# bdwsq1996/Effi-MVS-plus

Measured on AMD Instinct MI355X. Metric: ref-views/sec (cost-volume hot path: warp + cost volume + 3-D regularisation + cascaded GRU refinement), higher is better.
Workload: dtype f32 (3x3 MFMA convs: products as 3 bf16 partial products hi*hi+hi*lo+lo*hi, f32 accumulate; all else f32); 1 GPU; cfg3: DTU-shaped 1600x1184, N=5 views (S=4 sources), 3-stage cascade ndepths=48,8,8, GRU iters 3,3,3, seeded-random weights, features of the stock FPN resident in HBM; parallelism=single GPU, views_in_flight=3, arithmetic=split

## Files before the change

### effi_mvs_plus_amd/csrc/api.hip

```cpp
#include "common.hpp"
#include <cstdlib>
#include <cstring>
#include <mutex>

extern "C" int effi_version(void) { return 200; }

extern "C" const char* effi_error_string(int code) {
    switch (code) {
        case EFFI_OK: return "ok";
        case EFFI_ERR_BADARG: return "bad argument (null pointer, non-positive size, or inconsistent shapes)";
        case EFFI_ERR_UNSUPPORTED: return "shape / channel count not instantiated in this build";
        case EFFI_ERR_LAUNCH: return "kernel launch failed (hipPeekAtLastError)";
        case EFFI_ERR_WORKSPACE: return "no workspace registered for the current device (effi_set_workspace)";
        default: return "unknown error code";
    }
}

static const void* g_workspace[EFFI_MAX_DEVICES];

extern "C" long effi_workspace_bytes(void) { return 256; }

extern "C" int effi_set_workspace(int device, void* workspace, long bytes) {
    if (device < 0 || device >= EFFI_MAX_DEVICES) return EFFI_ERR_BADARG;
    if (workspace != nullptr && bytes < effi_workspace_bytes()) return EFFI_ERR_BADARG;
    __atomic_store_n(&g_workspace[device], (const void*)workspace, __ATOMIC_RELEASE);
    return EFFI_OK;
}

extern "C" const void* effi_get_workspace(int device) {
    if (device < 0 || device >= EFFI_MAX_DEVICES) return nullptr;
    return __atomic_load_n(&g_workspace[device], __ATOMIC_ACQUIRE);
}

const float* effi_zero_page() {
    int dev = -1;
    if (hipGetDevice(&dev) != hipSuccess) return nullptr;
    return (const float*)effi_get_workspace(dev);
}

namespace {
const char* const kOptName[EFFI_OPT_COUNT] = {"warp_lds_kb", "dyn_form", "dyn_setup_exact", "dyn_xchg", "pixnet_mfma", "force_mr", "mr4_min",
                                              "mr4_nt2_max", "mr2_min", "wide_tiles", "roll_mr", "roll_zt", "roll_rp", "deconv_mr", "sr_waves", "enc_gen_mr3", "c3_lean", "dyn_win"};
long g_opt[EFFI_OPT_COUNT];
std::once_flag g_opt_once;
void load_options() {
    for (int i = 0; i < EFFI_OPT_COUNT; ++i) {
        char env[64] = "EFFI_";
        size_t n = strlen(env);
        for (const char* c = kOptName[i]; *c && n + 1 < sizeof(env); ++c) env[n++] = (*c >= 'a' && *c <= 'z') ? (char)(*c - 32) : *c;
        env[n] = 0;
        const char* v = getenv(env);
        g_opt[i] = (v && *v) ? atol(v) : EFFI_OPT_UNSET;
    }
}
int find_option(const char* name) {
    if (!name) return -1;
    for (int i = 0; i < EFFI_OPT_COUNT; ++i)
        if (strcmp(name, kOptName[i]) == 0) return i;
    return -1;
}
}

long effi_option(int id) {
    std::call_once(g_opt_once, load_options);
    return __atomic_load_n(&g_opt[id], __ATOMIC_RELAXED);
}

extern "C" int effi_set_option(const char* name, long value) {
    const int id = find_option(name);
    if (id < 0) return EFFI_ERR_BADARG;
    std::call_once(g_opt_once, load_options);
    __atomic_store_n(&g_opt[id], value, __ATOMIC_RELAXED);
    return EFFI_OK;
}

extern "C" long effi_get_option(const char* name) {
    const int id = find_option(name);
    return id < 0 ? EFFI_OPT_UNSET : effi_option(id);
}

extern "C" long effi_option_unset(void) { return EFFI_OPT_UNSET; }

namespace {
__global__ __launch_bounds__(256) void lds_poison_kernel(unsigned pattern, unsigned* sink) {
    __shared__ unsigned buf[16 * 1024];
    for (int i = threadIdx.x; i < 16 * 1024; i += 256) buf[i] = pattern;
    __syncthreads();
    if (buf[(threadIdx.x * 61) & 16383] != pattern) sink[0] = 1;
}
}

extern "C" int effi_debug_poison_lds(unsigned pattern, void* sink4, effi_stream_t stream) {
    if (!sink4) return EFFI_ERR_BADARG;
    hipLaunchKernelGGL(lds_poison_kernel, dim3(2048), dim3(256), 0, effi_s(stream), pattern, reinterpret_cast<unsigned*>(sink4));
    EFFI_LAUNCH_CHECK();
// ... 63 lines not shown
```

### effi_mvs_plus_amd/csrc/common.hpp

```cpp
#pragma once
#include <hip/hip_runtime.h>
#include "../../include/effi_mvs_hip.h"

#define EFFI_LAUNCH_CHECK()                                   \
    do {                                                      \
        if (hipPeekAtLastError() != hipSuccess) return EFFI_ERR_LAUNCH; \
    } while (0)

const float* effi_zero_page();

enum EffiOption {
    EFFI_OPT_WARP_LDS_KB,
    EFFI_OPT_DYN_FORM,
    EFFI_OPT_DYN_SETUP_EXACT,
    EFFI_OPT_DYN_XCHG,
    EFFI_OPT_PIXNET_MFMA,
    EFFI_OPT_FORCE_MR,
    EFFI_OPT_MR4_MIN, EFFI_OPT_MR4_NT2_MAX, EFFI_OPT_MR2_MIN,
    EFFI_OPT_WIDE_TILES,
    EFFI_OPT_ROLL_MR, EFFI_OPT_ROLL_ZT, EFFI_OPT_ROLL_RP,
    EFFI_OPT_DECONV_MR,
    EFFI_OPT_SR_WAVES,
    EFFI_OPT_ENC_GEN_MR3,
    EFFI_OPT_C3_LEAN,
    EFFI_OPT_DYN_WIN,
    EFFI_OPT_COUNT
};
constexpr long EFFI_OPT_UNSET = -0x7fffffffL;
long effi_option(int id);

static inline hipStream_t effi_s(effi_stream_t s) {
    (void)hipGetLastError();
    return reinterpret_cast<hipStream_t>(s);
}
static inline int effi_cdiv(long a, long b) { return (int)((a + b - 1) / b); }

struct EffiPtrList {
    const float* p[EFFI_MAX_VIEWS + 1];
    const float* const* tbl;
};
__device__ __forceinline__ const float* effi_resolve_views(const float* ref, const EffiPtrList& l) {
    return l.tbl ? l.tbl[0] : ref;
}
struct EffiOutList {
    float* p[EFFI_MAX_VIEWS + 1];
};

__device__ __forceinline__ float effi_dpp_f(float v, int ctrl_sel) {
    int i = __float_as_int(v);
    int r;
    switch (ctrl_sel) {
        case 0:  r = __builtin_amdgcn_update_dpp(0, i, 0xB1, 0xF, 0xF, true); break;
        case 1:  r = __builtin_amdgcn_update_dpp(0, i, 0x4E, 0xF, 0xF, true); break;
        default: r = __builtin_amdgcn_update_dpp(0, i, 0x141, 0xF, 0xF, true); break;
    }
    return __int_as_float(r);
}

template <int LPP>
__device__ __forceinline__ float effi_group_sum(float v) {
    static_assert(LPP == 1 || LPP == 2 || LPP == 4 || LPP == 8, "lanes per pixel");
    if (LPP >= 2) v += effi_dpp_f(v, 0);
    if (LPP >= 4) v += effi_dpp_f(v, 1);
    if (LPP >= 8) v += effi_dpp_f(v, 2);
    return v;
}
template <int LPP>
__device__ __forceinline__ float effi_group_max(float v) {
    if (LPP >= 2) v = fmaxf(v, effi_dpp_f(v, 0));
    if (LPP >= 4) v = fmaxf(v, effi_dpp_f(v, 1));
    if (LPP >= 8) v = fmaxf(v, effi_dpp_f(v, 2));
    return v;
}

__device__ __forceinline__ int effi_xcd_remap(int bid, int nblocks) {
    const int q = nblocks >> 3, r = nblocks & 7;
    const int xcd = bid & 7, idx = bid >> 3;
    const int base = (xcd < r) ? xcd * (q + 1) : r * (q + 1) + (xcd - r) * q;
// ... 307 lines not shown
```

### effi_mvs_plus_amd/csrc/conv2d_x3.hpp

```cpp
#pragma once
#include "common.hpp"

#ifdef EFFI_BF16_ONLY
#define EFFI_FN(name) name##_bf16
#else
#define EFFI_FN(name) name
#endif

#ifndef EFFI_ABL
#define EFFI_ABL 0
#endif
#ifndef EFFI_PIPE_FRAGS
#define EFFI_PIPE_FRAGS 0
#endif

#ifndef EFFI_EPI_BATCH
#define EFFI_EPI_BATCH 1
#endif
#ifndef EFFI_EPI_EARLY_MAX
#define EFFI_EPI_EARLY_MAX 16
#endif
#ifndef EFFI_B_EARLY
#define EFFI_B_EARLY 0
#endif
// ... 152 lines not shown
        }
#pragma unroll
        for (int r = 0; r < 4; ++r) dst[(long)r * hw] = effi_sigmoid_split(v[r]) * (is_z ? 1.0f : hv[r]);
    } else if (EPI == EFFI_EPI_GRU_Q) {
        if (nvalid <= 0) return;
        if (SR && a.aux_q4) {
            const long oq = ((long)(co0 >> 2) * hw + pix) * 4;
            const f32x4 h4 = *reinterpret_cast<const f32x4*>(a.aux0 + oq), z4 = *reinterpret_cast<const f32x4*>(a.aux1 + oq);
            f32x4 g;
#pragma unroll
            for (int r = 0; r < 4; ++r) g[r] = (1.0f - z4[r]) * h4[r] + z4[r] * effi_tanh_split(v[r]);
            *reinterpret_cast<f32x4*>(a.out0 + oq) = g;
            effi_sr_store4(a.out_sr, a.sr_hp, a.sr_wp, co0, y, x, g);
            return;
        }
        const long o = (long)co0 * hw + pix;
        float hv[4], zv[4];
#pragma unroll
        for (int r = 0; r < 4; ++r) {
            hv[r] = a.aux0[o + (long)r * hw];
            zv[r] = a.aux1[o + (long)r * hw];
        }
        f32x4 g;
#pragma unroll
        for (int r = 0; r < 4; ++r) g[r] = (1.0f - zv[r]) * hv[r] + zv[r] * effi_tanh_split(v[r]);
#pragma unroll
        for (int r = 0; r < 4; ++r) a.out0[o + (long)r * hw] = g[r];
        if (SR) effi_sr_store4(a.out_sr, a.sr_hp, a.sr_wp, co0, y, x, g);
    }
}

typedef __bf16 bf16x8 __attribute__((ext_vector_type(8)));

#define EFFI_EPI_K1 6
#define EFFI_EPI_K1UP 8
#define EFFI_EPI_K1HEAD 7
typedef __bf16 bf16x2 __attribute__((ext_vector_type(2)));
typedef float f32x2 __attribute__((ext_vector_type(2)));

__device__ __forceinline__ void split_octet(const f32x4 (&pa)[8], int px, bf16x8& hi, bf16x8& lo) {
#pragma unroll
    for (int e = 0; e < 8; e += 2) {
        const f32x2 x = {pa[e][px], pa[e + 1][px]};
        const bf16x2 h2 = __builtin_convertvector(x, bf16x2);
        const f32x2 hf = __builtin_convertvector(h2, f32x2);
        const bf16x2 l2 = __builtin_convertvector(x - hf, bf16x2);
        hi[e] = h2[0];
        hi[e + 1] = h2[1];
        lo[e] = l2[0];
        lo[e + 1] = l2[1];
    }
}

template <int NT, int MR, int EPI, bool ZB, bool WIDE, bool SR = false, int NW = 4, bool GEN = false, bool REMAP = true>
__device__ __forceinline__ void conv2d_k3_bf16x3_tile(const Conv2dArgs a, int tiles_x, int ntiles, int bid, int nbid, int bidy,
                                                      const EncGenArgs* gp = nullptr, int gmode = 0) {
    constexpr int NTHR = NW * 64;
    static_assert(!GEN || SR, "generated inputs use the split-resident LDS image");
    static_assert(NW == 4 || (SR && NW == 8), "eight waves: split-resident kernels only");
    constexpr int TR = WIDE ? NW : NW * MR, TW = WIDE ? 16 * MR : 16;
    constexpr int AR = TR + 2, AW = SR ? TW + 2 : TW + 8, AQ = AW / 4, XOFF = SR ? 0 : 3, XLEFT = 4, CCH = 16, NKS = 5;
    constexpr int MROW = WIDE ? 0 : AW * 8, MCOL = WIDE ? 16 * 8 : 0;
    constexpr int APIX = AR * AW, NITEMS = (APIX / 4) * 2;
    constexpr int APIXP = SR ? ((APIX + 15) & ~15) : APIX;
    constexpr int NPART = kHiOnly ? 1 : 2;
    constexpr int NUA = SR ? (NPART * 2 * APIXP + NTHR - 1) / NTHR : 1;
    constexpr int NBF = NKS * NT * 2 * 64;
    constexpr int NB4 = (NBF + NTHR - 1) / NTHR;
    static_assert(SR || NITEMS <= 256, "one staging item per thread");
    static_assert(!(SR && ZB), "split-resident maps are 2-D");
    static_assert(EPI != EFFI_EPI_HEAD && EPI != EFFI_EPI_ADD_UP2, "epilogue not instantiated for the split-precision kernel");
    static_assert((EPI != EFFI_EPI_K1 && EPI != EFFI_EPI_K1UP && EPI != EFFI_EPI_K1HEAD) || !ZB, "the fused 1x1 epilogue is 2-D only");
    constexpr bool kHead = EPI == EFFI_EPI_K1HEAD;
    static_assert(!kHead || (SR && !WIDE && !GEN), "the one-launch depth head reads split-resident maps on 16-column tiles");
    __shared__ __attribute__((aligned(16))) unsigned short lds_ah[SR ? NUA * NTHR * 8 : APIX * CCH];
    __shared__ __attribute__((aligned(16))) unsigned short lds_al[SR ? 8 : APIX * CCH];
    __shared__ __attribute__((aligned(16))) unsigned short lds_b[NB4 * NTHR * 8];
    const unsigned short* const lds_al_rd = SR ? lds_ah + 2 * APIXP * 8 : lds_al;
    constexpr int IW7 = (AW + 7 + 1) & ~1, IH7 = AR + 7;
    __shared__ float lds_inv[GEN ? IH7 * IW7 : 1];

    const int tid = threadIdx.x, lane = tid & 63, wv = tid >> 6;
    const int li = lane & 15, lk = lane >> 4;
    const int h = a.h, w = a.w;
    const long hw = (long)h * w;
    const int tile = REMAP ? effi_xcd_remap(bid, nbid) : bid;
    if (tile >= ntiles) return;
    const int ty_ = tile / tiles_x;
    const int x0 = kHead ? (tile - ty_ * tiles_x) * (TW - 2) - 1 : (tile - ty_ * tiles_x) * TW, y0 = kHead ? ty_ * (TR - 2) - 1 : ty_ * TR;
    const int zpl = ZB ? bidy : 0;

    const bool stager = tid < NITEMS;
    const int pq = stager ? tid % (APIX / 4) : 0, soct = stager ? tid / (APIX / 4) : 0;
    const int srow = pq / AQ, sqx = pq - srow * AQ;
    const int sgy = y0 - 1 + srow, sgx = x0 - XLEFT + 4 * sqx;
    const bool s_in = stager & (sgy >= 0) & (sgy < h) & (sgx >= 0) & (sgx < w);
    const int s_off = sgy * w + sgx;
    const int s_lds = (soct * APIX + srow * AW + 4 * sqx) * 8;
    const int s_nv = w - sgx;
    const bool s_part = s_nv < 4;

    f32x4 pa[SR ? NUA : 8];
    const int cin_eff = ZB ? 3 * a.cin : a.cin;
    const int nchunks = (cin_eff + CCH - 1) / CCH;
    const unsigned short* wbf = reinterpret_cast<const unsigned short*>(a.wpack);
    int goff[NUA];
    if (SR && !GEN) {
#pragma unroll
        for (int j = 0; j < NUA; ++j) {
            const int u = tid + j * NTHR;
// ... 111 lines not shown
                    if (!kHiOnly) *reinterpret_cast<effi_bf16x8_t*>(&lds_ah[((1 * 2 + oct) * APIXP + p) * 8]) = lo;
                }
            }
        }
        if (GEN && gmode != 0) {
            const EncGenArgs& g = *gp;
            const int hd = g.hd;
            effi_bf16x8_t wh[2], wl[2];
#pragma unroll
            for (int s_ = 0; s_ < 2; ++s_) {
                const int ky = 4 * s_ + lk;
                float wv8[8];
#pragma unroll
                for (int kx = 0; kx < 8; ++kx) wv8[kx] = (ky < 7 && kx < 7) ? g.w_d1[(ky * 7 + kx) * hd + CCH * ch + li] : 0.0f;
                effi_split8(wv8, wh[s_], wl[s_]);
            }
            float b4[4];
#pragma unroll
            for (int r = 0; r < 4; ++r) b4[r] = g.b_d1[CCH * ch + 4 * lk + r];
            constexpr int NSEG = (APIX + 15) / 16;
            for (int seg = wv; seg < NSEG; seg += NW) {
                const int pr = seg * 16 + li, p = min(pr, APIX - 1);
                const int row = p / AW, col = p - row * AW;
                const int gy = y0 - 1 + row, gx = x0 - 1 + col;
                const bool inside = (gy >= 0) & (gy < h) & (gx >= 0) & (gx < w);
                f32x4 acc = {0.0f, 0.0f, 0.0f, 0.0f};
#pragma unroll
                for (int s_ = 0; s_ < 2; ++s_) {
                    const float* rowp = lds_inv + (row + 4 * s_ + lk) * IW7 + col;
                    float x8[8];
#pragma unroll
                    for (int i = 0; i < 8; ++i) x8[i] = rowp[i];
                    effi_bf16x8_t ah, al;
                    effi_split8(x8, ah, al);
                    acc = __builtin_amdgcn_mfma_f32_16x16x32_bf16(wh[s_], ah, acc, 0, 0, 0);
                    acc = __builtin_amdgcn_mfma_f32_16x16x32_bf16(wl[s_], ah, acc, 0, 0, 0);
                    acc = __builtin_amdgcn_mfma_f32_16x16x32_bf16(wh[s_], al, acc, 0, 0, 0);
                }
                f32x4 v;
#pragma unroll
                for (int r = 0; r < 4; ++r) v[r] = inside ? fmaxf(acc[r] + b4[r], 0.0f) : 0.0f;
                const bf16x4 h4 = __builtin_convertvector(v, bf16x4);
                const bf16x4 l4 = __builtin_convertvector(v - __builtin_convertvector(h4, f32x4), bf16x4);
                if (pr < APIX) {
                    const int e = ((lk >> 1) * APIXP + p) * 8 + (lk & 1) * 4;
                    *reinterpret_cast<bf16x4*>(&lds_ah[e]) = h4;
                    if (!kHiOnly) *reinterpret_cast<bf16x4*>(&lds_ah[2 * APIXP * 8 + e]) = l4;
                }
            }
        }
    };

    f32x4 tb[NB4];
    auto fetch_b = [&](int ch) {
#pragma unroll
        for (int j = 0; j < NB4; ++j) {
            const int u = min(tid + j * NTHR, NBF - 1);
            tb[j] = *reinterpret_cast<const f32x4*>(wbf + ((long)ch * NBF + u) * 8);
        }
    };
    constexpr bool kBEarly = SR && !GEN && EFFI_B_EARLY;
    auto stash = [&](int ch) {
        if (!kBEarly || ch == 0) fetch_b(ch);
        if constexpr (GEN) {
            generate(ch);
        } else if constexpr (SR) {
#pragma unroll
            for (int j = 0; j < NUA; ++j) *reinterpret_cast<f32x4*>(&lds_ah[(tid + j * NTHR) * 8]) = pa[j];
        } else if (stager) {
#pragma unroll
            for (int px = 0; px < 4; ++px) {
                bf16x8 hi, lo;
                split_octet(pa, px, hi, lo);
                *reinterpret_cast<bf16x8*>(&lds_ah[s_lds + px * 8]) = hi;
                if (!kHiOnly) *reinterpret_cast<bf16x8*>(&lds_al[s_lds + px * 8]) = lo;
            }
        }
#pragma unroll
        for (int j = 0; j < NB4; ++j) *reinterpret_cast<f32x4*>(&lds_b[(tid + j * NTHR) * 8]) = tb[j];
    };

    int koff[NKS];
#pragma unroll
    for (int s_ = 0; s_ < NKS; ++s_) {
        const int item = 4 * s_ + lk;
        const int tap = min(item >> 1, 8), oct = item & 1;
        koff[s_] = (((WIDE ? wv : wv * MR) + tap / 3) * AW + li + XOFF + tap % 3 + oct * APIXP) * 8;
    }

    f32x4 acc[MR][NT];
#pragma unroll
    for (int m = 0; m < MR; ++m)
#pragma unroll
        for (int n = 0; n < NT; ++n) acc[m][n] = f32x4{0.0f, 0.0f, 0.0f, 0.0f};

    constexpr bool kBatchT = SR && EFFI_EPI_BATCH != 0 && !(EFFI_ABL & 24) &&
                             (EPI == EFFI_EPI_PLAIN || EPI == EFFI_EPI_GRU_ZR || EPI == EFFI_EPI_GRU_Q);
    constexpr int NZ = (EPI == EFFI_EPI_GRU_ZR) ? NT / 2 : 0;
    constexpr int NH = !kBatchT ? 0 : (EPI == EFFI_EPI_GRU_ZR ? NT - NZ : (EPI == EFFI_EPI_GRU_Q ? NT : 0));
    constexpr int NZQ = (kBatchT && EPI == EFFI_EPI_GRU_Q) ? NT : 0;
    constexpr bool kStateEarly = MR * (NH + NZQ) * 4 <= EFFI_EPI_EARLY_MAX;
    const bool ebatch = kBatchT && (EPI == EFFI_EPI_PLAIN || a.aux_q4);
    f32x4 eb[kBatchT ? NT : 1], eh[MR][NH > 0 ? NH : 1], ez[MR][NZQ > 0 ? NZQ : 1];
    unsigned eqb[MR];
    bool einside[MR];
    auto epi_issue_bias = [&]() {
        if (!ebatch) return;
#pragma unroll
        for (int n = 0; n < NT; ++n) eb[n] = *reinterpret_cast<const f32x4*>(a.bias + n * 16 + 4 * lk);
#pragma unroll
        for (int m = 0; m < MR; ++m) {
            const int x = x0 + li + (WIDE ? 16 * m : 0), y = y0 + (WIDE ? wv : wv * MR + m);
            einside[m] = (y < h) & (x < w);
            eqb[m] = ((unsigned)lk * (unsigned)hw + (einside[m] ? (unsigned)(y * w + x) : 0u)) * 4u;
        }
    };
    auto epi_issue_state = [&]() {
        if (!ebatch) return;
#pragma unroll
        for (int m = 0; m < MR; ++m) {
#pragma unroll
            for (int j = 0; j < NH; ++j) eh[m][j] = *reinterpret_cast<const f32x4*>(a.aux0 + (size_t)(eqb[m] + (unsigned)j * 16u * (unsigned)hw));
#pragma unroll
            for (int j = 0; j < NZQ; ++j) ez[m][j] = *reinterpret_cast<const f32x4*>(a.aux1 + (size_t)(eqb[m] + (unsigned)j * 16u * (unsigned)hw));
        }
    };

    constexpr bool kK1 = (EPI == EFFI_EPI_K1 || EPI == EFFI_EPI_K1UP || kHead) && !(EFFI_ABL & 24) && EFFI_EPI_BATCH != 0;
    f32x4 kb[kK1 ? NT : 1], kex[kK1 ? MR : 1];
    if constexpr (kK1) {
#pragma unroll
        for (int n = 0; n < NT; ++n) kb[n] = *reinterpret_cast<const f32x4*>(a.bias + n * 16 + 4 * lk);
#pragma unroll
        for (int m = 0; m < MR; ++m) kex[m] = f32x4{0.0f, 0.0f, 0.0f, 0.0f};
        if (EPI == EFFI_EPI_K1 && a.hd > 0) {
#pragma unroll
            for (int m = 0; m < MR; ++m) {
                const int x = x0 + li + (WIDE ? 16 * m : 0), y = y0 + (WIDE ? wv : wv * MR + m);
                const unsigned pix = ((y < h) & (x < w)) ? (unsigned)(y * w + x) : 0u;
#pragma unroll
                for (int r = 0; r < 4; ++r) {
                    const int c = 4 * lk + r;
                    const float t_ = a.aux0[(size_t)((unsigned)min(c, a.hd - 1) * (unsigned)hw + pix)];
                    kex[m][r] = (c < a.hd) ? t_ : 0.0f;
                }
            }
        }
    }

    constexpr bool kBiasQ = !kBatchT && !kK1 && !(EFFI_ABL & 24) && EFFI_EPI_BATCH != 0;
    f32x4 gb[kBiasQ ? NT : 1];
    if constexpr (kBiasQ) {
#pragma unroll
        for (int n = 0; n < NT; ++n) gb[n] = *reinterpret_cast<const f32x4*>(a.bias + n * 16 + 4 * lk);
    }

    prefetch(0);
    epi_issue_bias();
    if (kStateEarly) epi_issue_state();
    stash(0);
    __syncthreads();
    for (int ch = 0; ch < nchunks; ++ch) {
        if (ch + 1 < nchunks) {
            prefetch(ch + 1);
            if (kBEarly) fetch_b(ch + 1);
        }
        constexpr int PIPE = SR ? EFFI_PIPE_FRAGS : 0;
        constexpr int MF = (PIPE == 2) ? (MR + 1) / 2 : MR, MB = MR - MF;
        bf16x8 ahf[PIPE ? 2 : 1][MF], alf[PIPE ? 2 : 1][MF], ahk[MB > 0 ? MB : 1], alk[MB > 0 ? MB : 1], bhb[NT], blb[NT];
        auto load_front = [&](int s_, int buf) {
#pragma unroll
            for (int m = 0; m < MF; ++m) {
                ahf[buf][m] = *reinterpret_cast<const bf16x8*>(&lds_ah[koff[s_] + m * (MROW + MCOL)]);
                if (!kHiOnly) alf[buf][m] = *reinterpret_cast<const bf16x8*>(&lds_al_rd[koff[s_] + m * (MROW + MCOL)]);
            }
        };
        auto load_back = [&](int s_) {
// ... 242 lines not shown
        for (int t = 0; t < nt2; ++t) {
            bf16x4 wh[NT + 1], wl[NT + 1];
#pragma unroll
            for (int n = 0; n <= NT; ++n) {
                const long f = ((long)(t * (NT + 1) + n) * 2) * 64 + lane;
                wh[n] = *reinterpret_cast<const bf16x4*>(w2 + f * 4);
                wl[n] = *reinterpret_cast<const bf16x4*>(w2 + (f + 64) * 4);
            }
            const int co = t * 16 + 4 * lk;
            float b2[4];
#pragma unroll
            for (int r = 0; r < 4; ++r) b2[r] = a.disp_range[co + r];
#pragma unroll
            for (int m = 0; m < MR; ++m) {
                f32x4 o = {0.0f, 0.0f, 0.0f, 0.0f};
#pragma unroll
                for (int n = 0; n <= NT; ++n) {
                    o = __builtin_amdgcn_mfma_f32_16x16x16bf16_1k(wh[n], xh[m][n], o, 0, 0, 0);
                    if (!kHiOnly) {
                        o = __builtin_amdgcn_mfma_f32_16x16x16bf16_1k(wl[n], xh[m][n], o, 0, 0, 0);
                        o = __builtin_amdgcn_mfma_f32_16x16x16bf16_1k(wh[n], xl[m][n], o, 0, 0, 0);
                    }
                }
                if (inside[m]) {
                    f32x4 vo;
#pragma unroll
                    for (int r = 0; r < 4; ++r) {
                        float v = o[r] + b2[r];
                        if (a.act == EFFI_ACT_RELU) v = fmaxf(v, 0.0f);
                        vo[r] = v;
                    }
                    if (SR && a.out_sr) {
                        effi_sr_store4(a.out_sr, a.sr_hp, a.sr_wp, co, y0 + (WIDE ? wv : wv * MR + m), x0 + li + (WIDE ? 16 * m : 0), vo);
                    } else {
#pragma unroll
                        for (int r = 0; r < 4; ++r)
                            if (co + r < a.n_range) a.out0[(long)(co + r) * hw + pixm[m]] = vo[r];
                    }
                }
            }
        }
        return;
    }
    if constexpr (kBatchT) if (ebatch) {
        if (!kStateEarly) epi_issue_state();
        const unsigned plane = (unsigned)a.sr_hp * (unsigned)a.sr_wp;
#pragma unroll
        for (int m = 0; m < MR; ++m) {
            if (!einside[m]) continue;
            const int x = x0 + li + (WIDE ? 16 * m : 0), y = y0 + (WIDE ? wv : wv * MR + m);
            const unsigned ub = (unsigned)lk * plane + (unsigned)(y + 1) * (unsigned)a.sr_wp + (unsigned)(x + 1);
#pragma unroll
            for (int n = 0; n < NT; ++n) {
                f32x4 v;
#pragma unroll
                for (int r = 0; r < 4; ++r) v[r] = acc[m][n][r] + eb[n][r];
                if constexpr (EPI == EFFI_EPI_PLAIN) {
                    if (a.act == EFFI_ACT_RELU) {
#pragma unroll
                        for (int r = 0; r < 4; ++r) v[r] = fmaxf(v[r], 0.0f);
                    } else if (a.act != EFFI_ACT_NONE) {
#pragma unroll
                        for (int r = 0; r < 4; ++r) v[r] = apply_act(v[r], a.act);
                    }
                    effi_sr_store4_at(a.out_sr, ub + (unsigned)(4 * n) * plane, lk & 1, v);
                    if (a.out0) {
                        float* dst = a.out0 + (long)(n * 16 + 4 * lk) * a.ostride + (long)y * w + x;
#pragma unroll
                        for (int r = 0; r < 4; ++r) dst[(long)r * a.ostride] = v[r];
                    }
                } else if constexpr (EPI == EFFI_EPI_GRU_ZR) {
                    f32x4 g;
                    if (n < NZ) {
#pragma unroll
                        for (int r = 0; r < 4; ++r) g[r] = effi_sigmoid_split(v[r]) * 1.0f;
                        *reinterpret_cast<f32x4*>(a.out0 + (size_t)(eqb[m] + (unsigned)n * 16u * (unsigned)hw)) = g;
                    } else {
#pragma unroll
                        for (int r = 0; r < 4; ++r) g[r] = effi_sigmoid_split(v[r]) * eh[m][n >= NZ ? n - NZ : 0][r];
                        effi_sr_store4_at(a.out_sr, ub + (unsigned)(4 * (n - NZ)) * plane, lk & 1, g);
                    }
                } else {
                    f32x4 g;
#pragma unroll
                    for (int r = 0; r < 4; ++r) g[r] = (1.0f - ez[m][n][r]) * eh[m][n][r] + ez[m][n][r] * effi_tanh_split(v[r]);
                    *reinterpret_cast<f32x4*>(a.out0 + (size_t)(eqb[m] + (unsigned)n * 16u * (unsigned)hw)) = g;
                    effi_sr_store4_at(a.out_sr, ub + (unsigned)(4 * n) * plane, lk & 1, g);
                }
            }
        }
        return;
    }
#pragma unroll
    for (int m = 0; m < MR; ++m) {
        const int x = x0 + li + (WIDE ? 16 * m : 0);
        const int y = y0 + (WIDE ? wv : wv * MR + m);
        if (y >= h || x >= w) continue;
        const long pix = (long)y * w + x;
#pragma unroll
        for (int n = 0; n < NT; ++n)
            conv_epilogue_store_t<((EPI == EFFI_EPI_K1 || EPI == EFFI_EPI_K1UP || EPI == EFFI_EPI_K1HEAD) ? EFFI_EPI_PLAIN : EPI), SR>(a, acc[m][n], n * 16 + 4 * lk, pix, hw, zpl, y, x,
                                                                                                          kBiasQ ? &gb[n] : nullptr);
    }
}

template <int NT, int MR, int EPI, bool ZB = false, bool WIDE = false, bool SR = false, int NW = 4>
__global__ __launch_bounds__(NW * 64) void conv2d_k3_bf16x3_kernel(const Conv2dArgs a, int tiles_x, int ntiles) {
#ifdef EFFI_STAGGER
    if (SR && gridDim.x > 512) {
        const int slot = (blockIdx.x >> 8) % 3;
        for (int i = 0; i < slot * EFFI_STAGGER; ++i) __builtin_amdgcn_s_sleep(127);
    }
#endif
    conv2d_k3_bf16x3_tile<NT, MR, EPI, ZB, WIDE, SR, NW>(a, tiles_x, ntiles, blockIdx.x, gridDim.x, blockIdx.y);
}

template <int NT, int MR, bool WIDE, bool SR = false, int NW = 4>
__global__ __launch_bounds__(NW * 64) void conv2d_k3_bf16x3_pair_kernel(const Conv2dArgs a0, const Conv2dArgs a1, int tiles_x, int ntiles) {
    if (blockIdx.y == 0) conv2d_k3_bf16x3_tile<NT, MR, EFFI_EPI_PLAIN, false, WIDE, SR, NW>(a0, tiles_x, ntiles, blockIdx.x, gridDim.x, 0);
    else conv2d_k3_bf16x3_tile<NT, MR, EFFI_EPI_PLAIN, false, WIDE, SR, NW>(a1, tiles_x, ntiles, blockIdx.x, gridDim.x, 0);
}

template <int NT, int MR, int EPI, bool WIDE>
__global__ __launch_bounds__(256) void conv2d_k3_bf16x3_batch_kernel(const Conv2dArgs a, const ConvBatch b, int tiles_x, int ntiles) {
    const int t = effi_xcd_remap(blockIdx.y * gridDim.x + blockIdx.x, gridDim.x * gridDim.y);
    const int img = t / ntiles;
    conv2d_k3_bf16x3_tile<NT, MR, EPI, false, WIDE, false, 4, false, false>(conv_batch_image(a, b, img), tiles_x, ntiles, t - img * ntiles,
                                                                           ntiles, 0);
}

template <int NT, int MR, bool WIDE>
__global__ __launch_bounds__(256) void conv2d_k3_bf16x3_encgen_pair_kernel(const Conv2dArgs a0, const Conv2dArgs a1, const EncGenArgs g,
                                                                           int tiles_x, int ntiles) {
    conv2d_k3_bf16x3_tile<NT, MR, EFFI_EPI_PLAIN, false, WIDE, true, 4, true>(blockIdx.y == 0 ? a0 : a1, tiles_x, ntiles, blockIdx.x, gridDim.x, 0, &g,
                                                                             (int)blockIdx.y);
}

static long effi_opt_or(int id, long dflt) {
    const long v = effi_option(id);
    return v == EFFI_OPT_UNSET ? dflt : v;
}
static long effi_mr4_min() { return effi_opt_or(EFFI_OPT_MR4_MIN, 400); }
static long effi_mr4_nt2_max() { return effi_opt_or(EFFI_OPT_MR4_NT2_MAX, 1024); }
static long effi_mr2_min() { return effi_opt_or(EFFI_OPT_MR2_MIN, 400); }
template <int NT, int EPI, bool ZB = false, bool SR = false>
static int launch_bf16x3(const Conv2dArgs& a, hipStream_t st) {
    const long cols = effi_cdiv(a.w, 16);
    const long planes = ZB ? a.zcount : 1;
    const long t4 = cols * effi_cdiv(a.h, 16) * planes, t2 = cols * effi_cdiv(a.h, 8) * planes;
    int mr;
    if (t4 >= effi_mr4_min() && !(NT == 2 && t4 >= effi_mr4_nt2_max())) mr = 4;
    else if (t2 >= effi_mr2_min()) mr = 2;
    else mr = 1;
    const long force = effi_opt_or(EFFI_OPT_FORCE_MR, 0);
    if (force) mr = (int)force;
    const long wide_env = effi_opt_or(EFFI_OPT_WIDE_TILES, -1);
    const bool wide = wide_env >= 0 ? wide_env != 0 : (mr == 4 && a.w >= 512 && !ZB);
    if (wide) {
        const int tiles_x = effi_cdiv(a.w, 16 * mr), ntiles = tiles_x * effi_cdiv(a.h, 4);
        const dim3 grid(ntiles, (unsigned)planes);
        if (mr == 4) hipLaunchKernelGGL((conv2d_k3_bf16x3_kernel<NT, 4, EPI, ZB, true, SR>), grid, dim3(256), 0, st, a, tiles_x, ntiles);
        else if (mr == 2) hipLaunchKernelGGL((conv2d_k3_bf16x3_kernel<NT, 2, EPI, ZB, true, SR>), grid, dim3(256), 0, st, a, tiles_x, ntiles);
        else hipLaunchKernelGGL((conv2d_k3_bf16x3_kernel<NT, 1, EPI, ZB, true, SR>), grid, dim3(256), 0, st, a, tiles_x, ntiles);
        return hipPeekAtLastError() == hipSuccess ? EFFI_OK : EFFI_ERR_LAUNCH;
    }
    if constexpr (SR) {
        const long srw = effi_option(EFFI_OPT_SR_WAVES);
        if ((srw == 8 && mr <= 2) || (srw == EFFI_OPT_UNSET && mr == 1 && NT >= 6)) {
            const int tiles_x = (int)cols, ntiles = tiles_x * effi_cdiv(a.h, 8 * mr);
            const dim3 grid(ntiles, 1);
            if (mr == 2) hipLaunchKernelGGL((conv2d_k3_bf16x3_kernel<NT, 2, EPI, false, false, true, 8>), grid, dim3(512), 0, st, a, tiles_x, ntiles);
            else hipLaunchKernelGGL((conv2d_k3_bf16x3_kernel<NT, 1, EPI, false, false, true, 8>), grid, dim3(512), 0, st, a, tiles_x, ntiles);
            return hipPeekAtLastError() == hipSuccess ? EFFI_OK : EFFI_ERR_LAUNCH;
        }
    }
    const int tiles_x = (int)cols, ntiles = tiles_x * effi_cdiv(a.h, 4 * mr);
    const dim3 grid(ntiles, (unsigned)planes);
    if (mr == 4) hipLaunchKernelGGL((conv2d_k3_bf16x3_kernel<NT, 4, EPI, ZB, false, SR>), grid, dim3(256), 0, st, a, tiles_x, ntiles);
    else if (mr == 2) hipLaunchKernelGGL((conv2d_k3_bf16x3_kernel<NT, 2, EPI, ZB, false, SR>), grid, dim3(256), 0, st, a, tiles_x, ntiles);
    else hipLaunchKernelGGL((conv2d_k3_bf16x3_kernel<NT, 1, EPI, ZB, false, SR>), grid, dim3(256), 0, st, a, tiles_x, ntiles);
    return hipPeekAtLastError() == hipSuccess ? EFFI_OK : EFFI_ERR_LAUNCH;
}

template <int NT, int EPI>
static int launch_bf16x3_batch(const Conv2dArgs& a, const ConvBatch& b, hipStream_t st) {
    const long cols = effi_cdiv(a.w, 16);
    const long t4 = cols * effi_cdiv(a.h, 16) * b.n_img, t2 = cols * effi_cdiv(a.h, 8) * b.n_img;
    int mr;
    if (t4 >= effi_mr4_min() && !(NT == 2 && t4 >= effi_mr4_nt2_max())) mr = 4;
    else if (t2 >= effi_mr2_min()) mr = 2;
    else mr = 1;
    const long force = effi_opt_or(EFFI_OPT_FORCE_MR, 0);
    if (force) mr = (int)force;
    if (mr != 1 && mr != 2 && mr != 4) return EFFI_ERR_BADARG;
    const long wide_env = effi_opt_or(EFFI_OPT_WIDE_TILES, -1);
    const bool wide = wide_env >= 0 ? wide_env != 0 : (mr == 4 && a.w >= 512);
    const int tiles_x = wide ? effi_cdiv(a.w, 16 * mr) : (int)cols, ntiles = tiles_x * effi_cdiv(a.h, wide ? 4 : 4 * mr);
    const dim3 grid(ntiles, (unsigned)b.n_img);
    if (wide) {
        if (mr == 4) hipLaunchKernelGGL((conv2d_k3_bf16x3_batch_kernel<NT, 4, EPI, true>), grid, dim3(256), 0, st, a, b, tiles_x, ntiles);
        else if (mr == 2) hipLaunchKernelGGL((conv2d_k3_bf16x3_batch_kernel<NT, 2, EPI, true>), grid, dim3(256), 0, st, a, b, tiles_x, ntiles);
        else hipLaunchKernelGGL((conv2d_k3_bf16x3_batch_kernel<NT, 1, EPI, true>), grid, dim3(256), 0, st, a, b, tiles_x, ntiles);
    } else {
        if (mr == 4) hipLaunchKernelGGL((conv2d_k3_bf16x3_batch_kernel<NT, 4, EPI, false>), grid, dim3(256), 0, st, a, b, tiles_x, ntiles);
        else if (mr == 2) hipLaunchKernelGGL((conv2d_k3_bf16x3_batch_kernel<NT, 2, EPI, false>), grid, dim3(256), 0, st, a, b, tiles_x, ntiles);
        else hipLaunchKernelGGL((conv2d_k3_bf16x3_batch_kernel<NT, 1, EPI, false>), grid, dim3(256), 0, st, a, b, tiles_x, ntiles);
    }
    return hipPeekAtLastError() == hipSuccess ? EFFI_OK : EFFI_ERR_LAUNCH;
}

template <int NT, int MR>
__global__ __launch_bounds__(256) void conv3d_k3_bf16x3_zb_batch_kernel(const Conv2dArgs a, const ConvBatch b, int tiles_x, int ntiles) {
    conv2d_k3_bf16x3_tile<NT, MR, EFFI_EPI_PLAIN, true, false, false, 4>(conv_batch_image(a, b, blockIdx.z), tiles_x, ntiles, blockIdx.x,
                                                                         gridDim.x, blockIdx.y);
}
template <int NT>
static int launch_bf16x3_zb_batch(const Conv2dArgs& a, const ConvBatch& b, hipStream_t st) {
    const long cols = effi_cdiv(a.w, 16), planes = (long)a.zcount * b.n_img;
    const long t4 = cols * effi_cdiv(a.h, 16) * planes, t2 = cols * effi_cdiv(a.h, 8) * planes;
    int mr;
// ... 104 lines not shown
```

### effi_mvs_plus_amd/ops.py

```python
from __future__ import annotations

import ctypes as C
import functools
import os
import threading

import weakref

import torch

from . import _lib
from ._lib import EffiLibraryError, check

ACT_NONE, ACT_RELU, ACT_SIGMOID, ACT_TANH = 0, 1, 2, 3
EPI_PLAIN, EPI_GRU_ZR, EPI_GRU_Q, EPI_HEAD, EPI_ADD_UP2, EPI_NHWC = 0, 1, 2, 3, 4, 5
EPI_ADD_SHUF2, EPI_NHWC_ADD_SHUF2 = 9, 10
MAX_VIEWS = 12


class KernelProfile:

    def __init__(self, keys=None):
        self.keys = None if keys is None else set(keys)
        self.records = []
# ... 6 lines not shown
                out[key] = out.get(key, 0.0) + acc
                acc = 0.0
            else:
                acc += e0.elapsed_time(e1)
        return out

    def summary(self):
        torch.cuda.synchronize()
        out = {}
        for key, work, e0, e1 in self.records:
            if e0 is None:
                continue
            d = out.setdefault(key, {"launches": 0, "ms": 0.0, "flops": 0.0, "bytes": 0.0})
            d["launches"] += 1
            d["ms"] += e0.elapsed_time(e1)
            d["flops"] += work.get("flops", 0.0)
            d["bytes"] += work.get("bytes", 0.0)
        return out


_PROF = None

PRECISIONS = ("split", "fp32", "bf16")
_PRECISION = os.environ.get("EFFI_MVS_PRECISION", "split")
if _PRECISION not in PRECISIONS:
    raise ValueError(f"EFFI_MVS_PRECISION must be one of {PRECISIONS}, got {_PRECISION!r}")


def set_precision(mode):
    global _PRECISION
    if mode not in PRECISIONS:
        raise ValueError(f"precision must be one of {PRECISIONS}, got {mode!r}")
    _PRECISION = mode


def get_precision():
    return _PRECISION


def uses_split():
    return _PRECISION in ("split", "bf16")


def _x3(name):
    return getattr(_lib.lib(), name + "_bf16" if _PRECISION == "bf16" else name)


_PY_OPTION_DEFAULTS = {"warp_x3": 0, "state_q4": 1, "c1k7_mfma": 1, "k5s2_split": 1, "roll": 1, "conv3d_unaligned_split": 1, "conv3d_s2_split": 1, "fpn_conv0_fused": 1,
                       "fpn_split_head": 1, "csp_pair": 1, "head_taps": 1, "enc_tail": 0, "enc_gen": 1, "reduce_chunk": 2048, "gru_fused": 0, "csp_gen": 0,
                       "head_fused": 1, "head_fused_tile": 0, "clear_fused": 1, "setup_fused": 1, "conf_fused": 1,
                       "fpn_batch": 1}
_PY_OPTS = {k: int(os.environ.get("EFFI_" + k.upper(), v)) for k, v in _PY_OPTION_DEFAULTS.items()}
LIB_OPTIONS = ("warp_lds_kb", "dyn_form", "dyn_setup_exact", "dyn_xchg", "pixnet_mfma", "force_mr", "mr4_min", "mr4_nt2_max", "mr2_min",
               "wide_tiles", "roll_mr", "roll_zt", "roll_rp", "deconv_mr", "sr_waves", "enc_gen_mr3", "c3_lean", "dyn_win")


def option(name):
    return _PY_OPTS[name]


def get_option(name):
    if name in _PY_OPTS:
        return _PY_OPTS[name]
    if name not in LIB_OPTIONS:
        raise KeyError(name)
    L = _lib.lib()
    v = L.effi_get_option(name.encode())
    return None if v == L.effi_option_unset() else int(v)


def set_option(name, value):
    before = get_option(name)
    if name in _PY_OPTS:
        _PY_OPTS[name] = _PY_OPTION_DEFAULTS[name] if value is None else int(value)
    else:
        L = _lib.lib()
        check(L.effi_set_option(name.encode(), L.effi_option_unset() if value is None else int(value)), "effi_set_option")
    return before


class options:

    def __init__(self, **kw):
        self.kw, self.before = kw, {}

    def __enter__(self):
        for k, v in self.kw.items():
            self.before[k] = set_option(k, v)
        return self

    def __exit__(self, *exc):
        for k, v in self.before.items():
            set_option(k, v)
        return False


def set_profile(p):
    global _PROF
    _PROF = p


def get_profile():
    return _PROF


def _call(key, work, fn, *args):
    p = _PROF
# ... 2026 lines not shown
```

Before: 633.6 views/s.

## Split output-channel tiles across blocks for small split-resident GRU convs

After: 636.9 views/s (median of 6 runs). Within noise of the previous version (+0.5%).

```diff
diff --git a/effi_mvs_plus_amd/csrc/api.hip b/effi_mvs_plus_amd/csrc/api.hip
--- a/effi_mvs_plus_amd/csrc/api.hip
+++ b/effi_mvs_plus_amd/csrc/api.hip
@@ -40,7 +40,7 @@
 
 namespace {
 const char* const kOptName[EFFI_OPT_COUNT] = {"warp_lds_kb", "dyn_form", "dyn_setup_exact", "dyn_xchg", "pixnet_mfma", "force_mr", "mr4_min",
-                                              "mr4_nt2_max", "mr2_min", "wide_tiles", "roll_mr", "roll_zt", "roll_rp", "deconv_mr", "sr_waves", "enc_gen_mr3", "c3_lean", "dyn_win"};
+                                              "mr4_nt2_max", "mr2_min", "wide_tiles", "roll_mr", "roll_zt", "roll_rp", "deconv_mr", "sr_waves", "enc_gen_mr3", "c3_lean", "dyn_win", "sr_nsplit"};
 long g_opt[EFFI_OPT_COUNT];
 std::once_flag g_opt_once;
 void load_options() {
diff --git a/effi_mvs_plus_amd/csrc/common.hpp b/effi_mvs_plus_amd/csrc/common.hpp
--- a/effi_mvs_plus_amd/csrc/common.hpp
+++ b/effi_mvs_plus_amd/csrc/common.hpp
@@ -24,6 +24,7 @@
     EFFI_OPT_ENC_GEN_MR3,
     EFFI_OPT_C3_LEAN,
     EFFI_OPT_DYN_WIN,
+    EFFI_OPT_SR_NSPLIT,
     EFFI_OPT_COUNT
 };
 constexpr long EFFI_OPT_UNSET = -0x7fffffffL;
diff --git a/effi_mvs_plus_amd/csrc/conv2d_x3.hpp b/effi_mvs_plus_amd/csrc/conv2d_x3.hpp
--- a/effi_mvs_plus_amd/csrc/conv2d_x3.hpp
+++ b/effi_mvs_plus_amd/csrc/conv2d_x3.hpp
@@ -228,10 +228,14 @@
     }
 }
 
-template <int NT, int MR, int EPI, bool ZB, bool WIDE, bool SR = false, int NW = 4, bool GEN = false, bool REMAP = true>
+template <int NT, int MR, int EPI, bool ZB, bool WIDE, bool SR = false, int NW = 4, bool GEN = false, bool REMAP = true, int NTG = NT>
 __device__ __forceinline__ void conv2d_k3_bf16x3_tile(const Conv2dArgs a, int tiles_x, int ntiles, int bid, int nbid, int bidy,
-                                                      const EncGenArgs* gp = nullptr, int gmode = 0) {
+                                                      const EncGenArgs* gp = nullptr, int gmode = 0, int n0 = 0) {
     constexpr int NTHR = NW * 64;
+    constexpr bool kSplit = NTG != NT;
+    static_assert(!kSplit || (SR && !GEN && !ZB && !WIDE && NTG % NT == 0 &&
+                              (EPI == EFFI_EPI_PLAIN || EPI == EFFI_EPI_GRU_ZR || EPI == EFFI_EPI_GRU_Q)),
+                  "N-split: split-resident plain / GRU epilogues on 16-column tiles");
     static_assert(!GEN || SR, "generated inputs use the split-resident LDS image");
     static_assert(NW == 4 || (SR && NW == 8), "eight waves: split-resident kernels only");
     constexpr int TR = WIDE ? NW : NW * MR, TW = WIDE ? 16 * MR : 16;
@@ -449,11 +453,24 @@
     };
 
     f32x4 tb[NB4];
-    auto fetch_b = [&](int ch) {
+    int boff[kSplit ? NB4 : 1];
+    if constexpr (kSplit) {
 #pragma unroll
         for (int j = 0; j < NB4; ++j) {
             const int u = min(tid + j * NTHR, NBF - 1);
-            tb[j] = *reinterpret_cast<const f32x4*>(wbf + ((long)ch * NBF + u) * 8);
+            const int sn = u >> 7, ks = sn / NT;
+            boff[j] = ((ks * NTG + n0 + (sn - ks * NT)) << 7) + (u & 127);
+        }
+    }
+    auto fetch_b = [&](int ch) {
+#pragma unroll
+        for (int j = 0; j < NB4; ++j) {
+            if constexpr (kSplit) {
+                tb[j] = *reinterpret_cast<const f32x4*>(wbf + ((long)ch * (NKS * NTG * 2 * 64) + boff[j]) * 8);
+            } else {
+                const int u = min(tid + j * NTHR, NBF - 1);
+                tb[j] = *reinterpret_cast<const f32x4*>(wbf + ((long)ch * NBF + u) * 8);
+            }
         }
     };
     constexpr bool kBEarly = SR && !GEN && EFFI_B_EARLY;
@@ -493,8 +510,8 @@
 
     constexpr bool kBatchT = SR && EFFI_EPI_BATCH != 0 && !(EFFI_ABL & 24) &&
                              (EPI == EFFI_EPI_PLAIN || EPI == EFFI_EPI_GRU_ZR || EPI == EFFI_EPI_GRU_Q);
-    constexpr int NZ = (EPI == EFFI_EPI_GRU_ZR) ? NT / 2 : 0;
-    constexpr int NH = !kBatchT ? 0 : (EPI == EFFI_EPI_GRU_ZR ? NT - NZ : (EPI == EFFI_EPI_GRU_Q ? NT : 0));
+    constexpr int NZ = (EPI == EFFI_EPI_GRU_ZR) ? NTG / 2 : 0;
+    constexpr int NH = !kBatchT ? 0 : (EPI == EFFI_EPI_GRU_ZR ? (kSplit ? NT : NT - NZ) : (EPI == EFFI_EPI_GRU_Q ? NT : 0));
     constexpr int NZQ = (kBatchT && EPI == EFFI_EPI_GRU_Q) ? NT : 0;
     constexpr bool kStateEarly = MR * (NH + NZQ) * 4 <= EFFI_EPI_EARLY_MAX;
     const bool ebatch = kBatchT && (EPI == EFFI_EPI_PLAIN || a.aux_q4);
@@ -504,7 +521,7 @@
     auto epi_issue_bias = [&]() {
         if (!ebatch) return;
 #pragma unroll
-        for (int n = 0; n < NT; ++n) eb[n] = *reinterpret_cast<const f32x4*>(a.bias + n * 16 + 4 * lk);
+        for (int n = 0; n < NT; ++n) eb[n] = *reinterpret_cast<const f32x4*>(a.bias + (n0 + n) * 16 + 4 * lk);
 #pragma unroll
         for (int m = 0; m < MR; ++m) {
             const int x = x0 + li + (WIDE ? 16 * m : 0), y = y0 + (WIDE ? wv : wv * MR + m);
@@ -517,9 +534,17 @@
 #pragma unroll
         for (int m = 0; m < MR; ++m) {
 #pragma unroll
-            for (int j = 0; j < NH; ++j) eh[m][j] = *reinterpret_cast<const f32x4*>(a.aux0 + (size_t)(eqb[m] + (unsigned)j * 16u * (unsigned)hw));
-#pragma unroll
-            for (int j = 0; j < NZQ; ++j) ez[m][j] = *reinterpret_cast<const f32x4*>(a.aux1 + (size_t)(eqb[m] + (unsigned)j * 16u * (unsigned)hw));
+            for (int j = 0; j < NH; ++j) {
+                if constexpr (kSplit && EPI == EFFI_EPI_GRU_ZR) {
+                    const int t = n0 + j - NZ;
+                    eh[m][j] = f32x4{0.0f, 0.0f, 0.0f, 0.0f};
+                    if (t >= 0) eh[m][j] = *reinterpret_cast<const f32x4*>(a.aux0 + (size_t)(eqb[m] + (unsigned)t * 16u * (unsigned)hw));
+                } else {
+                    eh[m][j] = *reinterpret_cast<const f32x4*>(a.aux0 + (size_t)(eqb[m] + (unsigned)(n0 + j) * 16u * (unsigned)hw));
+                }
+            }
+#pragma unroll
+            for (int j = 0; j < NZQ; ++j) ez[m][j] = *reinterpret_cast<const f32x4*>(a.aux1 + (size_t)(eqb[m] + (unsigned)(n0 + j) * 16u * (unsigned)hw));
         }
     };
 
@@ -868,6 +893,7 @@
             const unsigned ub = (unsigned)lk * plane + (unsigned)(y + 1) * (unsigned)a.sr_wp + (unsigned)(x + 1);
 #pragma unroll
             for (int n = 0; n < NT; ++n) {
+                const int gn = kSplit ? n0 + n : n;
                 f32x4 v;
 #pragma unroll
                 for (int r = 0; r < 4; ++r) v[r] = acc[m][n][r] + eb[n][r];
@@ -879,29 +905,29 @@
 #pragma unroll
                         for (int r = 0; r < 4; ++r) v[r] = apply_act(v[r], a.act);
                     }
-                    effi_sr_store4_at(a.out_sr, ub + (unsigned)(4 * n) * plane, lk & 1, v);
+                    effi_sr_store4_at(a.out_sr, ub + (unsigned)(4 * gn) * plane, lk & 1, v);
                     if (a.out0) {
-                        float* dst = a.out0 + (long)(n * 16 + 4 * lk) * a.ostride + (long)y * w + x;
+                        float* dst = a.out0 + (long)(gn * 16 + 4 * lk) * a.ostride + (long)y * w + x;
 #pragma unroll
                         for (int r = 0; r < 4; ++r) dst[(long)r * a.ostride] = v[r];
                     }
                 } else if constexpr (EPI == EFFI_EPI_GRU_ZR) {
                     f32x4 g;
-                    if (n < NZ) {
+                    if (gn < NZ) {
 #pragma unroll
                         for (int r = 0; r < 4; ++r) g[r] = effi_sigmoid_split(v[r]) * 1.0f;
-                        *reinterpret_cast<f32x4*>(a.out0 + (size_t)(eqb[m] + (unsigned)n * 16u * (unsigned)hw)) = g;
+                        *reinterpret_cast<f32x4*>(a.out0 + (size_t)(eqb[m] + (unsigned)gn * 16u * (unsigned)hw)) = g;
                     } else {
 #pragma unroll
-                        for (int r = 0; r < 4; ++r) g[r] = effi_sigmoid_split(v[r]) * eh[m][n >= NZ ? n - NZ : 0][r];
-                        effi_sr_store4_at(a.out_sr, ub + (unsigned)(4 * (n - NZ)) * plane, lk & 1, g);
+                        for (int r = 0; r < 4; ++r) g[r] = effi_sigmoid_split(v[r]) * eh[m][kSplit ? n : (n >= NZ ? n - NZ : 0)][r];
+                        effi_sr_store4_at(a.out_sr, ub + (unsigned)(4 * (gn - NZ)) * plane, lk & 1, g);
                     }
                 } else {
                     f32x4 g;
 #pragma unroll
                     for (int r = 0; r < 4; ++r) g[r] = (1.0f - ez[m][n][r]) * eh[m][n][r] + ez[m][n][r] * effi_tanh_split(v[r]);
-                    *reinterpret_cast<f32x4*>(a.out0 + (size_t)(eqb[m] + (unsigned)n * 16u * (unsigned)hw)) = g;
-                    effi_sr_store4_at(a.out_sr, ub + (unsigned)(4 * n) * plane, lk & 1, g);
+                    *reinterpret_cast<f32x4*>(a.out0 + (size_t)(eqb[m] + (unsigned)gn * 16u * (unsigned)hw)) = g;
+                    effi_sr_store4_at(a.out_sr, ub + (unsigned)(4 * gn) * plane, lk & 1, g);
                 }
             }
         }
@@ -915,7 +941,7 @@
         const long pix = (long)y * w + x;
 #pragma unroll
         for (int n = 0; n < NT; ++n)
-            conv_epilogue_store_t<((EPI == EFFI_EPI_K1 || EPI == EFFI_EPI_K1UP || EPI == EFFI_EPI_K1HEAD) ? EFFI_EPI_PLAIN : EPI), SR>(a, acc[m][n], n * 16 + 4 * lk, pix, hw, zpl, y, x,
+            conv_epilogue_store_t<((EPI == EFFI_EPI_K1 || EPI == EFFI_EPI_K1UP || EPI == EFFI_EPI_K1HEAD) ? EFFI_EPI_PLAIN : EPI), SR>(a, acc[m][n], (n0 + n) * 16 + 4 * lk, pix, hw, zpl, y, x,
                                                                                                           kBiasQ ? &gb[n] : nullptr);
     }
 }
@@ -931,6 +957,15 @@
     conv2d_k3_bf16x3_tile<NT, MR, EPI, ZB, WIDE, SR, NW>(a, tiles_x, ntiles, blockIdx.x, gridDim.x, blockIdx.y);
 }
 
+template <int NT, int NTL, int MR, int EPI, int NW>
+__global__ __launch_bounds__(NW * 64) void conv2d_k3_bf16x3_nsplit_kernel(const Conv2dArgs a, int tiles_x, int ntiles) {
+    constexpr int NS = NT / NTL;
+    const int t = effi_xcd_remap(blockIdx.x, gridDim.x);
+    const int tile = t / NS;
+    conv2d_k3_bf16x3_tile<NTL, MR, EPI, false, false, true, NW, false, false, NT>(a, tiles_x, ntiles, tile, ntiles, 0, nullptr, 0,
+                                                                                 (t - tile * NS) * NTL);
+}
+
 template <int NT, int MR, bool WIDE, bool SR = false, int NW = 4>
 __global__ __launch_bounds__(NW * 64) void conv2d_k3_bf16x3_pair_kernel(const Conv2dArgs a0, const Conv2dArgs a1, int tiles_x, int ntiles) {
     if (blockIdx.y == 0) conv2d_k3_bf16x3_tile<NT, MR, EFFI_EPI_PLAIN, false, WIDE, SR, NW>(a0, tiles_x, ntiles, blockIdx.x, gridDim.x, 0);
@@ -959,6 +994,26 @@
 static long effi_mr4_min() { return effi_opt_or(EFFI_OPT_MR4_MIN, 400); }
 static long effi_mr4_nt2_max() { return effi_opt_or(EFFI_OPT_MR4_NT2_MAX, 1024); }
 static long effi_mr2_min() { return effi_opt_or(EFFI_OPT_MR2_MIN, 400); }
+template <int NT, int NTL, int EPI>
+static int launch_bf16x3_nsplit(const Conv2dArgs& a, int mr, int nw, hipStream_t st) {
+    const int tiles_x = effi_cdiv(a.w, 16), ntiles = tiles_x * effi_cdiv(a.h, nw * mr);
+    const dim3 grid((unsigned)ntiles * (NT / NTL), 1);
+    if (nw == 8 && mr == 1) hipLaunchKernelGGL((conv2d_k3_bf16x3_nsplit_kernel<NT, NTL, 1, EPI, 8>), grid, dim3(512), 0, st, a, tiles_x, ntiles);
+    else if (nw == 8 && mr == 2) hipLaunchKernelGGL((conv2d_k3_bf16x3_nsplit_kernel<NT, NTL, 2, EPI, 8>), grid, dim3(512), 0, st, a, tiles_x, ntiles);
+    else if (nw == 4 && mr == 1) hipLaunchKernelGGL((conv2d_k3_bf16x3_nsplit_kernel<NT, NTL, 1, EPI, 4>), grid, dim3(256), 0, st, a, tiles_x, ntiles);
+    else if (nw == 4 && mr == 2) hipLaunchKernelGGL((conv2d_k3_bf16x3_nsplit_kernel<NT, NTL, 2, EPI, 4>), grid, dim3(256), 0, st, a, tiles_x, ntiles);
+    else if (nw == 4 && mr == 4) hipLaunchKernelGGL((conv2d_k3_bf16x3_nsplit_kernel<NT, NTL, 4, EPI, 4>), grid, dim3(256), 0, st, a, tiles_x, ntiles);
+    else return EFFI_ERR_BADARG;
+    return hipPeekAtLastError() == hipSuccess ? EFFI_OK : EFFI_ERR_LAUNCH;
+}
+template <int NT, int EPI>
+static int dispatch_bf16x3_nsplit(const Conv2dArgs& a, int ns, int mr, int nw, hipStream_t st) {
+    if constexpr (NT % 2 == 0) if (ns == 2) return launch_bf16x3_nsplit<NT, NT / 2, EPI>(a, mr, nw, st);
+    if constexpr (NT % 3 == 0) if (ns == 3) return launch_bf16x3_nsplit<NT, NT / 3, EPI>(a, mr, nw, st);
+    if constexpr (NT == 4 || NT == 6) if (ns == NT) return launch_bf16x3_nsplit<NT, 1, EPI>(a, mr, nw, st);
+    return EFFI_ERR_BADARG;
+}
+
 template <int NT, int EPI, bool ZB = false, bool SR = false>
 static int launch_bf16x3(const Conv2dArgs& a, hipStream_t st) {
     const long cols = effi_cdiv(a.w, 16);
@@ -982,6 +1037,20 @@
     }
     if constexpr (SR) {
         const long srw = effi_option(EFFI_OPT_SR_WAVES);
+        if constexpr ((EPI == EFFI_EPI_PLAIN && NT == 3) || (EPI == EFFI_EPI_GRU_ZR && (NT == 2 || NT == 4 || NT == 6)) ||
+                      (EPI == EFFI_EPI_GRU_Q && (NT == 2 || NT == 3))) {
+            const long nso = effi_option(EFFI_OPT_SR_NSPLIT);
+            int ns = 0, smr = (mr == 4 || mr == 2) ? mr : 1, snw = ((srw == 8 && mr <= 2) || (srw == EFFI_OPT_UNSET && mr == 1 && NT >= 6)) ? 8 : 4;
+            if (nso != EFFI_OPT_UNSET) {
+                if (nso >= 2 && nso <= NT && NT % nso == 0) ns = (int)nso;
+            } else if (!force && srw == EFFI_OPT_UNSET) {
+                if (EPI == EFFI_EPI_GRU_ZR && NT == 6 && mr == 1 && t2 <= 256) ns = 3, smr = 2, snw = 4;
+                else if (EPI == EFFI_EPI_GRU_Q && NT == 3 && mr == 1 && t2 < 128) ns = 3, smr = 1, snw = 4;
+                else if (EPI == EFFI_EPI_GRU_Q && NT == 2 && mr == 4 && t4 < 512) ns = 2;
+                else if (EPI == EFFI_EPI_GRU_Q && NT == 2 && mr == 1 && t2 <= 256) ns = 2, smr = 2, snw = 4;
+            }
+            if (ns) return dispatch_bf16x3_nsplit<NT, EPI>(a, ns, smr, snw, st);
+        }
         if ((srw == 8 && mr <= 2) || (srw == EFFI_OPT_UNSET && mr == 1 && NT >= 6)) {
             const int tiles_x = (int)cols, ntiles = tiles_x * effi_cdiv(a.h, 8 * mr);
             const dim3 grid(ntiles, 1);
diff --git a/effi_mvs_plus_amd/ops.py b/effi_mvs_plus_amd/ops.py
--- a/effi_mvs_plus_amd/ops.py
+++ b/effi_mvs_plus_amd/ops.py
@@ -82,7 +82,7 @@
                        "fpn_batch": 1}
 _PY_OPTS = {k: int(os.environ.get("EFFI_" + k.upper(), v)) for k, v in _PY_OPTION_DEFAULTS.items()}
 LIB_OPTIONS = ("warp_lds_kb", "dyn_form", "dyn_setup_exact", "dyn_xchg", "pixnet_mfma", "force_mr", "mr4_min", "mr4_nt2_max", "mr2_min",
-               "wide_tiles", "roll_mr", "roll_zt", "roll_rp", "deconv_mr", "sr_waves", "enc_gen_mr3", "c3_lean", "dyn_win")
+               "wide_tiles", "roll_mr", "roll_zt", "roll_rp", "deconv_mr", "sr_waves", "enc_gen_mr3", "c3_lean", "dyn_win", "sr_nsplit")
 
 
 def option(name):
```
